# srv/pcl_feature_extraction

Hardware: AMD Instinct MI355X
Metric: Mpoints/s through NARF keypoint + FPFH descriptor on 1M-pt cloud (higher is better)
Workload: dtype f32; 1 GPU; configs[2] 1M-pt synthetic room, NARF(support 0.2) + normals(r 0.05) + FPFH(r 0.08) at the keypoints; image=640x480, parallelism=scan-per-gpu x1, descriptor_rows=83

## Files before the change

### pcl_feature_extraction_amd/csrc/pfx_nblist.hip

```cpp
#include <cstdlib>
#include <cstring>
#include <rocprim/rocprim.hpp>

#include "pfx_nblist.h"
#include "pfx_neighbors.h"

namespace pfx {
namespace {

constexpr int kQ = 16;
typedef float pf2 __attribute__((ext_vector_type(2)));
constexpr int kArena = 16384;
constexpr int kArenaQuery = 16384;
constexpr int kTcapSmall = 384, kTcapSparse = 1280, kTcapDense = 8000;
constexpr int kCapQuery = 4096, kBucketsQuery = 1024;
constexpr int kCapMid8 = 8192, kBucketsMid8 = 1024;
constexpr int kCapMid = 16384, kBucketsMid = 2048;
#ifndef PFX_HUGE_BLOCKS
#define PFX_HUGE_BLOCKS 1024
#endif
constexpr int kCapHuge = 1 << 18, kBucketsHuge = 4096, kHugeBlocks = PFX_HUGE_BLOCKS;
#ifndef PFX_NT_QUERY
#define PFX_NT_QUERY 512
#endif
#ifndef PFX_NT_MID
#define PFX_NT_MID 1024
#endif
#ifndef PFX_NT_MID8
#define PFX_NT_MID8 1024
#endif
#ifndef PFX_Q_PF
#define PFX_Q_PF 1
#endif
#ifndef PFX_Q_WPE
#define PFX_Q_WPE 6
#endif
constexpr int kNtQuery = PFX_NT_QUERY, kNtMid8 = PFX_NT_MID8, kNtMid = PFX_NT_MID, kNtHuge = 256;

enum Counter : int {
  kTilesSmall, kTilesSparse, kTilesDense, kTilesWide,
  kWork4k, kRetryFirst = kWork4k, kWork8k, kWork16k, kWorkHuge,
  kHeadSmall, kHeadSparse, kHeadDense, kHeadWide, kHead4k, kHead8k, kHead16k, kHeadHuge,
  kOverCap,
  kNCounters
};

enum RanTier : int { kRan8k = 1, kRan16k = 2, kRanWide = 4, kRanAll = kRan8k | kRan16k | kRanWide };

constexpr int kCUs = 256;
constexpr int kGridSmall = kCUs * 4 * 2;
constexpr int kGridSparse = kCUs * 3 * 4;
constexpr int kGridDense = kCUs * 2 * 4;
constexpr int kGridWide = kCUs * 4;
constexpr int kGrid4k = kCUs * 4;
constexpr int kGrid8k = kCUs * 2;
constexpr int kGrid16k = kCUs;
constexpr int kGridHugeMax = kHugeBlocks;
constexpr size_t kArenaTails = (size_t)(kGridSmall + kGridSparse + kGridDense) * kArena +
                               (size_t)(kGridWide + kGrid4k + kGrid8k + kGrid16k + kGridHugeMax) * kArenaQuery;

constexpr int32_t kListMode = 1 << 30;
struct TierQ {
  int32_t* q[4];
  int* n[4];
};
__device__ __forceinline__ int query_tier(int k) {
  return k <= kCapQuery ? 0 : (k <= kCapMid8 ? 1 : (k <= kCapMid ? 2 : 3));
}

constexpr int kRecInts = 24;
constexpr int kRecQ0 = 19, kRecQn = 20;

__device__ __forceinline__ void rec_write(int32_t* __restrict__ rec, const Runs& R, int32_t q0, int qn) {
#pragma unroll
  for (int r = 0; r < 9; ++r) rec[r] = R.start[r];
#pragma unroll
  for (int r = 0; r < 10; ++r) rec[9 + r] = R.pref[r];
  rec[kRecQ0] = q0;
  rec[kRecQn] = qn;
}

__device__ __forceinline__ int rec_load(const int32_t* __restrict__ rec_base, int rec_step, int i, bool ok) {
  const int lane = threadIdx.x & 63;
  return (ok && lane < kRecInts) ? rec_base[(int64_t)i * rec_step + lane] : 0;
}
// ... 257 lines not shown
      for (int idx = tid; idx < words; idx += 256) {
        const int tl = idx / kRecInts, w = idx - tl * kRecInts;
        const int32_t v = w < kRecQ0 ? s_runs[s_tcell[tl]][w] : (w == kRecQ0 ? s_tq0[tl] : (w == kRecQn ? s_tqn[tl] : 0));
        recs[(int64_t)s_tat[tl] * kRecInts + w] = v;
      }
      __syncthreads();
    }
  }
}

struct ListOut {
  int64_t* off;
  int32_t* cnt;
  uint8_t* lg;
  uint32_t* list;
  unsigned long long* cursor;
  unsigned long long cap;
  int compact;
  int32_t* qrec;
};

struct CandLds {
  const float2* cxy;
  const float* cz;
  __device__ __forceinline__ void get(int t, float& x, float& y, float& z) const {
    const float2 v = cxy[t];
    x = v.x; y = v.y; z = cz[t];
  }
};
struct CandGlobal {
  const float4* sp;
  const Runs* R;
  __device__ __forceinline__ void get(int t, float& x, float& y, float& z) const {
    const float4 c = sp[run_pos(*R, t)];
    x = c.x; y = c.y; z = c.z;
  }
};

#ifdef PFX_SHOT_PROFILE
constexpr int kTileProbes = 28, kWaveProbes = 12;
__device__ unsigned long long g_tile_prof[kTileProbes];
__device__ unsigned long long g_tile_prof2[kWaveProbes];
#define TPROF_DECL unsigned long long tacc_[kTileProbes] = {}, wacc_[kWaveProbes] = {}
#define TPROF_T(v) long long v = (threadIdx.x == 0) ? clock64() : 0
#define TPROF_ADD(i, a, b) tacc_[i] += (unsigned long long)((b) - (a))
#define WPROF_T(v) long long v = ((threadIdx.x & 63) == 0) ? clock64() : 0
#define WPROF_ADD(i, a, b) wacc_[i] += (unsigned long long)((b) - (a))
#define TPROF_FLUSH                                                                      \
  do {                                                                                   \
    if (threadIdx.x == 0)                                                                \
      _Pragma("unroll") for (int i_ = 0; i_ < kTileProbes; ++i_)                         \
        if (tacc_[i_]) atomicAdd(&g_tile_prof[i_], tacc_[i_]);                           \
    if ((threadIdx.x & 63) == 0)                                                         \
      _Pragma("unroll") for (int i_ = 0; i_ < kWaveProbes; ++i_)                         \
        if (wacc_[i_]) atomicAdd(&g_tile_prof2[i_], wacc_[i_]);                          \
  } while (0)
#else
#define TPROF_DECL
#define TPROF_T(v)
#define TPROF_ADD(i, a, b)
#define WPROF_T(v)
#define WPROF_ADD(i, a, b)
#define TPROF_FLUSH
#endif

template <int NB, int E, class Cand>
__device__ __forceinline__ void wave_sort_regs(uint16_t* L, int k, float qx, float qy, float qz, const Cand& cand,
                                               float bscale, uint32_t* Sd, uint16_t* St, int* bcount, int* bpos,
                                               const GridView& g, const Runs& R, int lane) {
  for (int b = lane; b < NB; b += 64) bcount[b] = 0;
  int t[E], b[E];
  uint32_t d[E];
#pragma unroll
  for (int i = 0; i < E; ++i) t[i] = lane + 64 * i < k ? L[lane + 64 * i] : 0;
  wave_sync();
#pragma unroll
  for (int i = 0; i < E; ++i) {
    float px, py, pz;
    cand.get(t[i], px, py, pz);
    const float d2 = flann_d2(qx, qy, qz, px, py, pz);
    d[i] = __float_as_uint(d2);
    const int bb = (int)(d2 * bscale);
    b[i] = bb < NB ? bb : NB - 1;
    if (lane + 64 * i < k) atomicAdd(&bcount[b[i]], 1);
  }
  wave_sync();
  {
    constexpr int PER = NB / 64;
    int c[PER], sum = 0;
#pragma unroll
    for (int v = 0; v < PER; ++v) { c[v] = bcount[lane * PER + v]; sum += c[v]; }
    const int inc = wave_incl_scan(sum);
    int ex = inc - sum;
#pragma unroll
    for (int v = 0; v < PER; ++v) { bpos[lane * PER + v] = ex; ex += c[v]; }
  }
  wave_sync();
  int slot[E];
#pragma unroll
  for (int i = 0; i < E; ++i) slot[i] = lane + 64 * i < k ? atomicAdd(&bpos[b[i]], 1) : 0;
#pragma unroll
  for (int i = 0; i < E; ++i)
    if (lane + 64 * i < k) {
      Sd[slot[i]] = d[i];
      St[slot[i]] = (uint16_t)t[i];
    }
  wave_sync();
  int st[E], en[E];
#pragma unroll
  for (int i = 0; i < E; ++i) {
    en[i] = bpos[b[i]];
    st[i] = en[i] - bcount[b[i]];
  }
  int rank[E];
  bool tie = false;
#pragma unroll
  for (int i = 0; i < E; ++i) {
    uint32_t dv[4];
#pragma unroll
    for (int j = 0; j < 4; ++j) dv[j] = st[i] + j < en[i] ? Sd[st[i] + j] : 0xffffffffu;
    int r = 0, eq = 0;
#pragma unroll
    for (int j = 0; j < 4; ++j) {
      r += dv[j] < d[i];
      eq += dv[j] == d[i];
    }
    for (int v = st[i] + 4; v < en[i]; ++v) {
      const uint32_t x = Sd[v];
      r += x < d[i];
      eq += x == d[i];
    }
    rank[i] = r;
    tie |= lane + 64 * i < k && eq > 1;
  }
  if (__builtin_amdgcn_ballot_w64(tie)) {
#pragma unroll
    for (int i = 0; i < E; ++i) {
      if (lane + 64 * i >= k) continue;
      const int32_t mine = g.perm[run_pos(R, t[i])];
      for (int v = st[i]; v < en[i]; ++v)
        if (v != slot[i] && Sd[v] == d[i] && g.perm[run_pos(R, St[v])] < mine) ++rank[i];
    }
  }
  wave_sync();
#pragma unroll
  for (int i = 0; i < E; ++i)
    if (lane + 64 * i < k) L[st[i] + rank[i]] = (uint16_t)t[i];
  wave_sync();
}

template <int NB, class Cand>
__device__ __forceinline__ void wave_sort(uint16_t* L, int k, float qx, float qy, float qz, const Cand& cand,
                                          float bscale, uint32_t* Sd, uint16_t* St, int* bcount, int* bpos,
                                          const GridView& g, const Runs& R, int lane) {
  for (int b = lane; b < NB; b += 64) bcount[b] = 0;
  wave_sync();
  for (int e = lane; e < k; e += 64) {
    const int t = L[e];
    float px, py, pz;
    cand.get(t, px, py, pz);
    const int b = (int)(flann_d2(qx, qy, qz, px, py, pz) * bscale);
    atomicAdd(&bcount[b < NB ? b : NB - 1], 1);
  }
  wave_sync();
  {
    constexpr int PER = NB / 64;
    int c[PER], s = 0;
#pragma unroll
    for (int v = 0; v < PER; ++v) { c[v] = bcount[lane * PER + v]; s += c[v]; }
    const int inc = wave_incl_scan(s);
    int ex = inc - s;
#pragma unroll
    for (int v = 0; v < PER; ++v) { bpos[lane * PER + v] = ex; ex += c[v]; }
  }
  wave_sync();
  for (int e = lane; e < k; e += 64) {
    const int t = L[e];
    float px, py, pz;
    cand.get(t, px, py, pz);
    const float d2 = flann_d2(qx, qy, qz, px, py, pz);
    int b = (int)(d2 * bscale);
    b = b < NB ? b : NB - 1;
    const int slot = atomicAdd(&bpos[b], 1);
    Sd[slot] = __float_as_uint(d2);
    St[slot] = (uint16_t)t;
  }
  wave_sync();
  auto bucket_rank = [&](int s, uint32_t d, int t, int st, int en) {
    uint32_t dv[4];
#pragma unroll
    for (int i = 0; i < 4; ++i) dv[i] = st + i < en ? Sd[st + i] : 0xffffffffu;
    int rank = 0;
#pragma unroll
    for (int i = 0; i < 4; ++i) {
      const int v = st + i;
      if (v < en) {
        if (dv[i] < d) ++rank;
        else if (dv[i] == d && v != s && g.perm[run_pos(R, St[v])] < g.perm[run_pos(R, t)]) ++rank;
      }
    }
    for (int v = st + 4; v < en; ++v) {
      const uint32_t x = Sd[v];
      if (x < d) ++rank;
      else if (x == d && v != s && g.perm[run_pos(R, St[v])] < g.perm[run_pos(R, t)]) ++rank;
    }
    return rank;
  };
  for (int s0 = lane; s0 < k; s0 += 128) {
    const int s1 = s0 + 64;
    const bool h1 = s1 < k;
    const uint32_t d0 = Sd[s0], d1 = h1 ? Sd[s1] : 0u;
    const int t0 = St[s0], t1 = h1 ? St[s1] : 0;
    int b0 = (int)(__uint_as_float(d0) * bscale), b1 = (int)(__uint_as_float(d1) * bscale);
    b0 = b0 < NB ? b0 : NB - 1;
    b1 = b1 < NB ? b1 : NB - 1;
    const int en0 = bpos[b0], c0 = bcount[b0], en1 = bpos[b1], c1 = bcount[b1];
    const int st0 = en0 - c0, st1 = en1 - c1;
    const int r0 = bucket_rank(s0, d0, t0, st0, en0);
    const int r1 = h1 ? bucket_rank(s1, d1, t1, st1, en1) : 0;
    L[st0 + r0] = (uint16_t)t0;
    if (h1) L[st1 + r1] = (uint16_t)t1;
  }
  wave_sync();
}

template <class Cand>
__device__ __forceinline__ void wave_rank_sort(uint16_t* L, int k, float qx, float qy, float qz, const Cand& cand,
                                               const GridView& g, const Runs& R, int lane) {
  const bool in = lane < k;
  const int t = in ? L[lane] : 0;
  float px, py, pz;
  cand.get(t, px, py, pz);
  const uint32_t d = in ? __float_as_uint(flann_d2(qx, qy, qz, px, py, pz)) : 0xffffffffu;
  int rank = 0, eq = 0;
  for (int m = 0; m < k; ++m) {
    const uint32_t dm = (uint32_t)__builtin_amdgcn_readlane((int)d, m);
    rank += dm < d ? 1 : 0;
    eq += dm == d ? 1 : 0;
  }
  if (__builtin_amdgcn_ballot_w64(in && eq > 1)) {
    const int32_t id = in ? g.perm[run_pos(R, t)] : 0x7fffffff;
    rank = 0;
    for (int m = 0; m < k; ++m) {
      const uint32_t dm = (uint32_t)__builtin_amdgcn_readlane((int)d, m);
      const int32_t im = __builtin_amdgcn_readlane(id, m);
      rank += (dm < d || (dm == d && im < id)) ? 1 : 0;
    }
  }
  wave_sync();
  if (in) L[rank] = (uint16_t)t;
  wave_sync();
}

template <int NB, class Cand, bool SMALL = false>
__device__ __forceinline__ void sort_list(uint16_t* L, int k, float qx, float qy, float qz, const Cand& cand,
                                          float bscale, uint32_t* Sd, uint16_t* St, int* bcount, int* bpos,
                                          const GridView& g, const Runs& R, int lane) {
  if (k <= 64) wave_rank_sort(L, k, qx, qy, qz, cand, g, R, lane);
  else if (k <= 128) wave_sort_regs<NB, 2>(L, k, qx, qy, qz, cand, bscale, Sd, St, bcount, bpos, g, R, lane);
  else if (k <= 192) wave_sort_regs<NB, 3>(L, k, qx, qy, qz, cand, bscale, Sd, St, bcount, bpos, g, R, lane);
  else if (k <= 256) wave_sort_regs<NB, 4>(L, k, qx, qy, qz, cand, bscale, Sd, St, bcount, bpos, g, R, lane);
  else if (k <= 320) wave_sort_regs<NB, 5>(L, k, qx, qy, qz, cand, bscale, Sd, St, bcount, bpos, g, R, lane);
  else if (SMALL || k <= 384) wave_sort_regs<NB, 6>(L, k, qx, qy, qz, cand, bscale, Sd, St, bcount, bpos, g, R, lane);
  else if (k <= 448) wave_sort_regs<NB, 7>(L, k, qx, qy, qz, cand, bscale, Sd, St, bcount, bpos, g, R, lane);
  else if (k <= 512) wave_sort_regs<NB, 8>(L, k, qx, qy, qz, cand, bscale, Sd, St, bcount, bpos, g, R, lane);
  else if (k <= 640) wave_sort_regs<NB, 10>(L, k, qx, qy, qz, cand, bscale, Sd, St, bcount, bpos, g, R, lane);
  else if (k <= 768) wave_sort_regs<NB, 12>(L, k, qx, qy, qz, cand, bscale, Sd, St, bcount, bpos, g, R, lane);
  else if (k <= 896) wave_sort_regs<NB, 14>(L, k, qx, qy, qz, cand, bscale, Sd, St, bcount, bpos, g, R, lane);
  else if (k <= 1024) wave_sort_regs<NB, 16>(L, k, qx, qy, qz, cand, bscale, Sd, St, bcount, bpos, g, R, lane);
  else wave_sort<NB>(L, k, qx, qy, qz, cand, bscale, Sd, St, bcount, bpos, g, R, lane);
}

__device__ __forceinline__ void push_sort(const TierQ* tq, int32_t j, int k) {
  const int t = query_tier(k);
  tq->q[t][atomicAdd(tq->n[t], 1)] = j | kListMode;
}

constexpr int kChunkWide = 1024;
template <bool STAGE, int SCAP, bool STORE>
__device__ __forceinline__ void tile_pass(const GridView& g, const Runs& R, int T, const float2* cxy, const float* cz,
                                          float2* hxy, float* hz, const pf2* qxy, const float* qz, const bool* act,
                                          const int64_t* gb, int* cursor, uint32_t* __restrict__ glist, float rr) {
  constexpr int CH = kChunkWide, U = 2, QW = 4;
  const int tid = threadIdx.x, lane = tid & 63;
#pragma unroll
  for (int u = 0; u < QW; ++u) cursor[u] = 0;
  float4 cc[STAGE ? 1 : CH / 256];
  if (!STAGE)
#pragma unroll
    for (int u = 0; u < CH / 256; ++u) cc[u] = g.sp[run_pos(R, min(tid + 256 * u, T - 1))];
  for (int c0 = 0; c0 < T; c0 += (STAGE ? T : CH)) {
    const int cend = STAGE ? T : min(T, c0 + CH);
    if (!STAGE) {
      __syncthreads();
#pragma unroll
      for (int u = 0; u < CH / 256; ++u) {
        hxy[tid + 256 * u] = make_float2(cc[u].x, cc[u].y);
        hz[tid + 256 * u] = cc[u].z;
      }
      __syncthreads();
      if (c0 + CH < T)
#pragma unroll
        for (int u = 0; u < CH / 256; ++u) cc[u] = g.sp[run_pos(R, min(c0 + CH + tid + 256 * u, T - 1))];
// ... 35 lines not shown
  }
}

template <int TCAP, bool STAGE>
struct Stager {
  static constexpr int PT = STAGE ? (TCAP + 255) / 256 : 0;
  float x[PT > 0 ? PT : 1], y[PT > 0 ? PT : 1], z[PT > 0 ? PT : 1];
  int32_t qp;
  __device__ __forceinline__ void load(const GridView& g, const int32_t* __restrict__ qpos, const Runs& R,
                                       int32_t start, int qn, bool ok) {
    const int tid = threadIdx.x;
    const int T = ok ? R.pref[9] : 0;
#pragma unroll
    for (int u = 0; u < PT; ++u) {
      const int tc = max(0, min(tid + 256 * u, T - 1));
      const float4 c = g.sp[run_pos(R, tc)];
      x[u] = c.x; y[u] = c.y; z[u] = c.z;
    }
    qp = qpos[start + (tid < qn ? tid : 0)];
  }
  __device__ __forceinline__ void store(float2* cxy, float* cz, int32_t* s_qp, int qn) const {
    const int tid = threadIdx.x;
#pragma unroll
    for (int u = 0; u < PT; ++u) {
      const int t = tid + 256 * u;
      cxy[t] = make_float2(x[u], y[u]);
      cz[t] = z[u];
    }
    if (tid < qn) s_qp[tid] = qp;
  }
};

template <int LCAP, int NB, int TCAP, bool STAGE>
__global__ void __launch_bounds__(256, TCAP <= kTcapSmall ? 4 : (STAGE ? 3 : 2)) k_nb_tile(GridView g, const int32_t* __restrict__ qpos,
                                                 const int32_t* __restrict__ rec_base, int rec_step,
                                                 const int* __restrict__ ntiles_ptr,
                                                 float rr, float bscale, int sorted, ListOut out,
                                                 const TierQ* __restrict__ tq,
                                                 int* __restrict__ next_tile, int chunk) {
  constexpr int Q = kQ, QW = Q / 4;
  constexpr int U = 2;
  constexpr int SCAP = STAGE ? Stager<TCAP, STAGE>::PT * 256 : 1;
  __shared__ float2 cxy[SCAP];
  __shared__ float cz[SCAP];
  constexpr int CH = STAGE ? 1 : 1024;
  __shared__ float2 hxy[CH];
  __shared__ float hz[CH];
  __shared__ uint16_t lists_flat[Q * (LCAP + 2) + 4 * 64];
  uint16_t(*lists)[LCAP + 2] = reinterpret_cast<uint16_t(*)[LCAP + 2]>(lists_flat);
  __shared__ uint32_t sd[4][LCAP];
  __shared__ uint16_t stt[4][LCAP];
  __shared__ int bcount[4][NB], bpos[4][NB];
  __shared__ int s_k[Q];
  __shared__ int32_t s_qp[Q];
  __shared__ unsigned long long s_base;
  __shared__ int s_chunk;
  const int tid = threadIdx.x, lane = tid & 63;
  const int wv = __builtin_amdgcn_readfirstlane(tid >> 6);
  const uint32_t trash_at = (uint32_t)(Q * (LCAP + 2) + 64 * wv + lane);
  const uint32_t wrow = (uint32_t)(wv * (LCAP + 2));
  const int ntiles = *ntiles_ptr;
  TPROF_DECL;
  unsigned long long wg_total = 0, arena_base = 0, arena_left = 0;
  int next_chunk = 0;
  if (tid == 0) {
    s_chunk = atomicAdd(next_tile, chunk);
    next_chunk = atomicAdd(next_tile, chunk);
  }
  __syncthreads();
  int i = __builtin_amdgcn_readfirstlane(s_chunk), i_end = i + chunk;
  Runs R;
  int32_t start = 0;
  int qn = 0;
  {
    const int v = rec_load(rec_base, rec_step, i, i < ntiles);
    rec_unpack(v, R, start, qn);
    Stager<TCAP, STAGE> sg;
    sg.load(g, qpos, R, start, qn, R.pref[9] <= TCAP);
    __syncthreads();
    if (i + 1 == i_end && tid == 0) {
      s_chunk = next_chunk;
      next_chunk = atomicAdd(next_tile, chunk);
    }
    sg.store(cxy, cz, s_qp, qn);
    __syncthreads();
  }
  while (i < ntiles) {
    TPROF_T(p0);
    const int T = R.pref[9];
    const bool ok = T <= TCAP;
    int ni = i + 1;
    if (ni == i_end) {
      ni = __builtin_amdgcn_readfirstlane(s_chunk);
      i_end = ni + chunk;
    }
    const int recv = rec_load(rec_base, rec_step, ni, ni < ntiles);
    pf2 qxy[QW];
    float qz[QW];
    int cursor[QW];
#pragma unroll
    for (int u = 0; u < QW; ++u) {
      const int j = wv + 4 * u;
      cursor[u] = 0;
      qxy[u] = pf2{0.f, 0.f};
      qz[u] = 0.f;
      if (j < qn) {
        const int32_t p = s_qp[j];
        if (STAGE) {
          const int t = R.pref[4] + (p - R.start[4]);
          const float2 v = cxy[t];
          qxy[u] = pf2{v.x, v.y};
          qz[u] = cz[t];
        } else {
          const float4 c = g.sp[p];
          qxy[u] = pf2{c.x, c.y};
          qz[u] = c.z;
        }
      }
    }
    for (int c0 = 0; ok && c0 < T; c0 += (STAGE ? T : CH)) {
      const int cend = STAGE ? T : min(T, c0 + CH);
      if (!STAGE) {
        constexpr int CPT = CH >= 256 ? CH / 256 : 1;
        float4 cc[CPT];
#pragma unroll
        for (int u = 0; u < CPT; ++u) cc[u] = g.sp[run_pos(R, min(c0 + tid + 256 * u, T - 1))];
        __syncthreads();
#pragma unroll
        for (int u = 0; u < CPT; ++u) {
          hxy[tid + 256 * u] = make_float2(cc[u].x, cc[u].y);
          hz[tid + 256 * u] = cc[u].z;
        }
        __syncthreads();
      }
      const float2* XYs = STAGE ? cxy : hxy - c0;
      const float* Zs = STAGE ? cz : hz - c0;
      for (int t0 = c0; t0 < cend; t0 += 64 * U) {
        pf2 pxy[U];
        float pz[U], rrv[U];
#pragma unroll
        for (int v = 0; v < U; ++v) {
          const int t = t0 + 64 * v + lane;
          const int tr = STAGE ? min(t, SCAP - 1) : t;
          const float2 xy = XYs[tr];
          pxy[v] = pf2{xy.x, xy.y};
          pz[v] = Zs[tr];
          rrv[v] = t < cend ? rr : -1.0f;
        }
#pragma unroll
// ... 12 lines not shown
                                                           __builtin_amdgcn_mbcnt_lo((uint32_t)m, (uint32_t)cursor[u]));
            const uint32_t hit_at = (uint32_t)(min(slot, LCAP) + wrow) + (uint32_t)(4 * u * (LCAP + 2));
            const uint32_t sel = 0u - (uint32_t)hit;
            lists_flat[trash_at ^ ((trash_at ^ hit_at) & sel)] = (uint16_t)t;
            cursor[u] += __popcll(m);
          }
        }
      }
    }
    if (lane == 0) {
#pragma unroll
      for (int u = 0; u < QW; ++u)
        if (wv + 4 * u < qn) {
          const int kq = ok ? cursor[u] : LCAP + 1;
          s_k[wv + 4 * u] = kq;
          if (kq > LCAP) qrec_write(out.qrec, start + wv + 4 * u, R, s_qp[wv + 4 * u], qxy[u].x, qxy[u].y, qz[u]);
        }
    }
    __syncthreads();
    TPROF_T(p1);
    TPROF_ADD(TCAP <= kTcapSmall ? 17 : (STAGE ? 1 : 5), p0, p1);
    WPROF_T(ws0);
    [[maybe_unused]] constexpr int kWp0 = TCAP <= kTcapSmall ? 0 : (STAGE ? 4 : 8);
    int lg = 0;
    while ((1 << lg) < qn) ++lg;
    bool c16 = out.compact != 0;
#pragma unroll
    for (int r = 0; r < 9; ++r) c16 = c16 && R.pref[r + 1] - R.pref[r] <= kCompactRun;
    int maxk = 0;
    for (int j = 0; j < qn; ++j) {
      const int k = s_k[j];
      maxk = (k <= LCAP && k > maxk) ? k : maxk;
    }
    if (tid == 0)
      for (int j = 0; j < qn; ++j) wg_total += s_k[j] <= LCAP ? (unsigned long long)s_k[j] : 0ull;
    const unsigned long long need = c16 ? (((unsigned long long)maxk << lg) + 1) >> 1 : (unsigned long long)maxk << lg;
    unsigned long long arena_new = 0, arena_res = 0;
    if (tid == 0 && need > arena_left) {
      arena_res = need > (unsigned long long)kArena ? need : (unsigned long long)kArena;
      arena_new = atomicAdd(out.cursor, arena_res);
    }
    if (tid < qn) {
      const int k = s_k[tid];
      if (k <= LCAP) {
        out.cnt[start + tid] = k;
        out.lg[start + tid] = (uint8_t)(lg | (c16 ? kLgCompact : 0));
      } else {
        const int t = ok ? query_tier(k) : 0;
        if (t == 0) tq->q[0][wave_push_slot(tq->n[0])] = start + tid;
        else tq->q[t][atomicAdd(tq->n[t], 1)] = start + tid;
      }
    }
    if (sorted) {
#pragma unroll
      for (int u = 0; u < QW; ++u) {
        const int j = wv + 4 * u;
        const int k = cursor[u];
        if (ok && j < qn && k <= LCAP && k > 1) {
          if (STAGE) {
            const CandLds cand{cxy, cz};
            sort_list<NB, CandLds, (TCAP <= kTcapSmall)>(lists[j], k, qxy[u].x, qxy[u].y, qz[u], cand, bscale, sd[wv],
                                                         stt[wv], bcount[wv], bpos[wv], g, R, lane);
          } else {
            const CandGlobal cand{g.sp, &R};
            sort_list<NB>(lists[j], k, qxy[u].x, qxy[u].y, qz[u], cand, bscale, sd[wv], stt[wv], bcount[wv], bpos[wv],
                          g, R, lane);
          }
        }
      }
    }
    WPROF_T(ws1);
    WPROF_ADD(kWp0 + 0, ws0, ws1);
    __syncthreads();
    TPROF_T(p2);
    TPROF_ADD(TCAP <= kTcapSmall ? 18 : (STAGE ? 2 : 6), p1, p2);
    WPROF_T(ws2);
    [[maybe_unused]] constexpr int kWp = TCAP <= kTcapSmall ? 0 : (STAGE ? 4 : 8);
    WPROF_ADD(kWp + 1, ws1, ws2);
    Runs Rn;
    int32_t start_n;
    int qn_n;
    rec_unpack(recv, Rn, start_n, qn_n);
    const bool ok_n = ni < ntiles && Rn.pref[9] <= TCAP;
    Stager<TCAP, STAGE> sg;
    if (ni < ntiles) sg.load(g, qpos, Rn, start_n, qn_n, ok_n);
    if (tid == 0) {
      if (ni + 1 == i_end) {
        s_chunk = next_chunk;
        next_chunk = atomicAdd(next_tile, chunk);
      }
      if (arena_res) {
        arena_base = arena_new;
        arena_left = arena_res;
      }
      s_base = arena_base;
      arena_base += need;
      arena_left -= need;
    }
    if (ni < ntiles) sg.store(cxy, cz, s_qp, qn_n);
    WPROF_T(ws3);
    WPROF_ADD(kWp + 2, ws2, ws3);
    __syncthreads();
    WPROF_T(ws4);
    const int64_t base = (int64_t)s_base;
    if (tid < qn && s_k[tid] <= LCAP) out.off[start + tid] = (c16 ? 2 * base : base) + tid;
    const int total = maxk << lg;
    if (c16) {
      const int words = (total + 1) >> 1;
      if ((unsigned long long)(base + words) <= out.cap) {
        for (int w = tid; w < words; w += 256) {
          uint32_t pair = 0;
#pragma unroll
          for (int h = 0; h < 2; ++h) {
            const int e = 2 * w + h;
            const int m = e >> lg, j = e & ((1 << lg) - 1);
            const int k = j < qn ? s_k[j] : 0;
            if (e < total && m < k && k <= LCAP) pair |= (uint32_t)run_entry16(R, lists[j][m]) << (16 * h);
          }
          out.list[base + w] = pair;
        }
      }
    } else if ((unsigned long long)(base + total) <= out.cap) {
      for (int e = tid; e < total; e += 256) {
        const int m = e >> lg, j = e & ((1 << lg) - 1);
        if (j < qn) {
          const int k = s_k[j];
          if (m < k && k <= LCAP) out.list[base + e] = run_entry(R, lists[j][m]);
        }
      }
    }
    WPROF_T(ws5);
    WPROF_ADD(kWp + 3, ws4, ws5);
    __syncthreads();
    TPROF_T(p3);
    TPROF_ADD(TCAP <= kTcapSmall ? 19 : (STAGE ? 3 : 7), p2, p3);
    i = ni;
    R = Rn;
    start = start_n;
    qn = qn_n;
  }
  if (tid == 0 && wg_total) atomicAdd(out.cursor + 1, wg_total);
  TPROF_FLUSH;
}

__global__ void __launch_bounds__(256) k_nb_wide(GridView g, const int32_t* __restrict__ qpos,
                                                 const int32_t* __restrict__ recs, const int32_t* __restrict__ work,
                                                 const int* __restrict__ n_ptr, float rr, int sorted, ListOut out,
                                                 const TierQ* __restrict__ tq, int* __restrict__ next_work) {
  constexpr int QW = 4;
  __shared__ float2 hxy[kChunkWide];
  __shared__ float hz[kChunkWide];
  __shared__ int s_k[kQ];
  __shared__ int32_t s_qp[kQ];
  __shared__ int s_w;
  __shared__ unsigned long long s_base;
  const int tid = threadIdx.x, lane = tid & 63;
  const int wv = __builtin_amdgcn_readfirstlane(tid >> 6);
  const int count = *n_ptr;
  if (count == 0) return;
  unsigned long long wg_total = 0, wg_long = 0, wg_long_n = 0, arena_base = 0, arena_left = 0;
  for (;;) {
    if (tid == 0) s_w = atomicAdd(next_work, 1);
    __syncthreads();
    const int w = __builtin_amdgcn_readfirstlane(s_w);
    __syncthreads();
    if (w >= count) break;
    Runs R;
    int32_t start;
    int qn;
    rec_unpack(rec_load(recs, kRecInts, work[w], true), R, start, qn);
    const int T = R.pref[9];
    if (tid < qn) s_qp[tid] = qpos[start + tid];
    __syncthreads();
    pf2 qxy[QW];
// ... 457 lines not shown
      atomicAdd(out.cursor + 2, wg_long);
      atomicAdd(out.cursor + 3, wg_long_n);
    }
  }
  TPROF_FLUSH;
}

std::string bname(const char* tag, const char* what) { return std::string(tag) + "_" + what; }

struct ListsRb {
  int cnt[kNCounters];
  int oob;
  unsigned long long cur[4];
  int64_t nq;
};

const ListsRb* read_back(pfx_ctx* ctx, const void* counters, const void* cursor, const void* d_nq, const int* oob) {
  hipStream_t st = ctx->stream;
  ListsRb* rb = ctx->readback<ListsRb>();
  PFX_HIP(hipMemcpyAsync(rb->cnt, counters, sizeof(rb->cnt), hipMemcpyDeviceToHost, st));
  PFX_HIP(hipMemcpyAsync(rb->cur, cursor, sizeof(rb->cur), hipMemcpyDeviceToHost, st));
  PFX_HIP(hipMemcpyAsync(&rb->nq, d_nq, sizeof(int64_t), hipMemcpyDeviceToHost, st));
  rb->oob = 0;
  if (oob) PFX_HIP(hipMemcpyAsync(&rb->oob, oob, sizeof(int), hipMemcpyDeviceToHost, st));
  ctx->sync_spin(st);
  return rb;
}

[[noreturn]] void throw_over_cap(const char* tag, int k) {
  throw Error(PFX_ERR_CAPACITY, std::string(tag) + ": a query has " + std::to_string(k) + " neighbours (> " +
                                    std::to_string(kCapHuge) + " supported)");
}

void publish(pfx_ctx* ctx, const char* tag, const ListsRb& rb, size_t list_words, NbLists& out) {
  out.nq = rb.nq;
  out.nq_dev = nullptr;
  out.total = (int64_t)rb.cur[1];
  out.long_total = (int64_t)rb.cur[2];
  out.long_nq = (int64_t)rb.cur[3];
  out.slots = (int64_t)rb.cur[0];
  auto stat = [&](const char* what) -> int64_t& { return ctx->stats[std::string(tag) + what]; };
  stat("_tiles_small") = rb.cnt[kTilesSmall];
  stat("_tiles_sparse") = rb.cnt[kTilesSparse];
  stat("_tiles_dense") = rb.cnt[kTilesDense];
  stat("_wide") = rb.cnt[kTilesWide];
  stat("_single") = rb.cnt[kWork4k];
  stat("_mid8") = rb.cnt[kWork8k];
  stat("_mid") = rb.cnt[kWork16k];
  stat("_huge") = rb.cnt[kWorkHuge];
  stat("_slots") = (int64_t)rb.cur[0];
  stat("_list_words") = (int64_t)list_words;
}

struct TierHint {
  const char* key;
  RanTier bit;
  Counter work;
};
constexpr TierHint kTierHints[3] = {
    {"_hint_mid8", kRan8k, kWork8k}, {"_hint_mid", kRan16k, kWork16k}, {"_hint_wide", kRanWide, kTilesWide}};
int wanted_tiers(pfx_ctx* ctx, const char* tag) {
  int ran = 0;
  for (const TierHint& h : kTierHints) {
    const auto it = ctx->stats.find(std::string(tag) + h.key);
    if (it == ctx->stats.end() || it->second > 0) ran |= h.bit;
  }
  return ran;
}
void note_mid_tiers(pfx_ctx* ctx, const char* tag, const int* h_cnt) {
  for (const TierHint& h : kTierHints) {
    int64_t& v = ctx->stats[std::string(tag) + h.key];
    v = h_cnt[h.work] > 0 ? 16 : std::max<int64_t>(0, v - 1);
  }
}

#ifdef PFX_SHOT_PROFILE
void report_probes(const char* tag) {
  unsigned long long pr[kTileProbes];
  PFX_HIP(hipMemcpyFromSymbol(pr, HIP_SYMBOL(g_tile_prof), sizeof(pr)));
  fprintf(stderr, "%s wave_sort cycles (wave 0): count %llu scan %llu scatter %llu rank %llu\n", tag, pr[8],
          pr[9], pr[10], pr[11]);
  fprintf(stderr, "%s tile cycles: sparse stage %llu test %llu sort %llu write %llu | dense - %llu test %llu "
          "sort %llu write %llu | small - %llu test %llu sort %llu write %llu (cumulative)\n", tag, pr[0], pr[1], pr[2],
          pr[3], pr[4], pr[5], pr[6], pr[7], pr[16], pr[17], pr[18], pr[19]);
  fprintf(stderr, "%s query cycles: test %llu sort+write %llu | entries %llu candidates %llu\n", tag, pr[20],
          pr[21], pr[22], pr[23]);
  fprintf(stderr, "%s query 4k-tier phases: scan %llu scatter %llu rank+write %llu | list-mode items %llu\n", tag,
          pr[24], pr[25], pr[26], pr[27]);
  unsigned long long pw[kWaveProbes];
  PFX_HIP(hipMemcpyFromSymbol(pw, HIP_SYMBOL(g_tile_prof2), sizeof(pw)));
  fprintf(stderr, "%s wave cycles (sum over waves): small sort %llu sortwait %llu staging %llu listwrite %llu | "
          "sparse %llu %llu %llu %llu | dense %llu %llu %llu %llu\n", tag, pw[0], pw[1], pw[2], pw[3], pw[4], pw[5],
          pw[6], pw[7], pw[8], pw[9], pw[10], pw[11]);
  static const unsigned long long zw[kWaveProbes] = {};
  PFX_HIP(hipMemcpyToSymbol(HIP_SYMBOL(g_tile_prof2), zw, sizeof(zw)));
  static const unsigned long long zero[kTileProbes] = {};
  PFX_HIP(hipMemcpyToSymbol(HIP_SYMBOL(g_tile_prof), zero, sizeof(zero)));
}
#endif

struct ListBuild {
  pfx_ctx* ctx;
  const Grid& G;
  const char* tag;
  hipStream_t st;
  const int64_t n;
  const GridView g;
  const float rr;
  const int isort, compact;
  int32_t *qpos, *seg, *tiles, *recs, *wq, *qrec, *cnt;
  int32_t *q4k, *q8k, *q16k, *qhuge;
  int64_t *d_nq, *d_ntiles, *off;
  uint8_t *flags, *lgs;
  int* counters;
  unsigned long long* cursor;
  TierQ* tq_dev;
  size_t t1 = 0, t2 = 0, t3 = 0;
  void* tmp;
  DevBuf &lb, &hs;
  int ch_small, ch_sparse, ch_dense;
  static constexpr size_t kHugeSlice = sizeof(uint32_t) * 4 * (size_t)kCapHuge;

  DevBuf& buf(const char* what) { return ctx->bufs[bname(tag, what)]; }

  ListBuild(pfx_ctx* c, const Grid& grid, const char* t, double radius, bool sorted, bool compact_)
      : ctx(c), G(grid), tag(t), st(c->stream), n(grid.n), g(view(grid)), rr((float)(radius * radius)),
        isort(sorted ? 1 : 0), compact(compact_ ? 1 : 0), lb(buf("list")), hs(buf("scratch")) {
    qpos = buf("qpos").as<int32_t>(n);
    d_nq = buf("nq").as<int64_t>(1);
    flags = buf("flags").as<uint8_t>(n);
// ... 264 lines not shown
```

Baseline: 219.5 Mpoints/s.

## Shrink dense tile LDS and registers to run three workgroups per CU

The dense neighbour-list tile kernel now targets three resident workgroups per CU instead of two. To get there it overlays the list rows, candidate staging and sort scratch in one shared-memory union and drops the separate tag array and bcount/bpos pair in favour of one in-place bucket array. It also adds a lean register-sort variant that recomputes buckets instead of holding them, and moves query coordinates and arena bookkeeping into LDS. The cost is extra recomputation and LDS traffic, plus a riskier in-place sort, in exchange for more latency hiding; the old spill-style wave_sort path is removed and an occupancy query is added to the stats.

New measurement: 229.7 Mpoints/s, median of 6. 4.7% higher.

```diff
diff --git a/pcl_feature_extraction_amd/csrc/pfx_nblist.hip b/pcl_feature_extraction_amd/csrc/pfx_nblist.hip
--- a/pcl_feature_extraction_amd/csrc/pfx_nblist.hip
+++ b/pcl_feature_extraction_amd/csrc/pfx_nblist.hip
@@ -1,5 +1,8 @@
+#include <array>
 #include <cstdlib>
 #include <cstring>
+#include <map>
+#include <mutex>
 #include <rocprim/rocprim.hpp>
 
 #include "pfx_nblist.h"
@@ -35,6 +38,13 @@
 #ifndef PFX_Q_WPE
 #define PFX_Q_WPE 6
 #endif
+#ifndef PFX_DENSE_WG_PER_CU
+#define PFX_DENSE_WG_PER_CU 3
+#endif
+#ifndef PFX_DENSE_ROUNDS
+#define PFX_DENSE_ROUNDS (PFX_DENSE_WG_PER_CU == 2 ? 4 : 2)
+#endif
+static_assert(PFX_DENSE_WG_PER_CU == 2 || PFX_DENSE_WG_PER_CU == 3, "the dense tiles run two or three workgroups per CU");
 constexpr int kNtQuery = PFX_NT_QUERY, kNtMid8 = PFX_NT_MID8, kNtMid = PFX_NT_MID, kNtHuge = 256;
 
 enum Counter : int {
@@ -48,9 +58,10 @@
 enum RanTier : int { kRan8k = 1, kRan16k = 2, kRanWide = 4, kRanAll = kRan8k | kRan16k | kRanWide };
 
 constexpr int kCUs = 256;
-constexpr int kGridSmall = kCUs * 4 * 2;
-constexpr int kGridSparse = kCUs * 3 * 4;
-constexpr int kGridDense = kCUs * 2 * 4;
+constexpr int kWgSmall = 4, kWgSparse = 3, kWgDense = PFX_DENSE_WG_PER_CU;
+constexpr int kGridSmall = kCUs * kWgSmall * 2;
+constexpr int kGridSparse = kCUs * kWgSparse * 4;
+constexpr int kGridDense = kCUs * kWgDense * PFX_DENSE_ROUNDS;
 constexpr int kGridWide = kCUs * 4;
 constexpr int kGrid4k = kCUs * 4;
 constexpr int kGrid8k = kCUs * 2;
@@ -374,7 +385,8 @@
   const float4* sp;
   const Runs* R;
   __device__ __forceinline__ void get(int t, float& x, float& y, float& z) const {
-    const float4 c = sp[run_pos(*R, t)];
+    typedef float pf3 __attribute__((ext_vector_type(3)));
+    const pf3 c = *reinterpret_cast<const pf3*>(sp + run_pos(*R, t));
     x = c.x; y = c.y; z = c.z;
   }
 };
@@ -406,12 +418,18 @@
 #define TPROF_FLUSH
 #endif
 
-template <int NB, int E, class Cand>
+template <int NB, int E, bool LEAN, class Cand>
 __device__ __forceinline__ void wave_sort_regs(uint16_t* L, int k, float qx, float qy, float qz, const Cand& cand,
-                                               float bscale, uint32_t* Sd, uint16_t* St, int* bcount, int* bpos,
-                                               const GridView& g, const Runs& R, int lane) {
-  for (int b = lane; b < NB; b += 64) bcount[b] = 0;
-  int t[E], b[E];
+                                               float bscale, uint32_t* Sd, int* bk, const GridView& g, const Runs& R,
+                                               int lane) {
+  auto bucket_of = [&](uint32_t dbits) {
+    const int bb = (int)(__uint_as_float(dbits) * bscale);
+    return bb < NB ? bb : NB - 1;
+  };
+  constexpr int EH = LEAN ? 1 : E;
+  for (int b = lane; b < NB; b += 64) bk[b] = 0;
+  int t[E];
+  [[maybe_unused]] int bh[EH], slot[EH], st[EH], en[EH];
   uint32_t d[E];
 #pragma unroll
   for (int i = 0; i < E; ++i) t[i] = lane + 64 * i < k ? L[lane + 64 * i] : 0;
@@ -420,149 +438,110 @@
   for (int i = 0; i < E; ++i) {
     float px, py, pz;
     cand.get(t[i], px, py, pz);
-    const float d2 = flann_d2(qx, qy, qz, px, py, pz);
-    d[i] = __float_as_uint(d2);
-    const int bb = (int)(d2 * bscale);
-    b[i] = bb < NB ? bb : NB - 1;
-    if (lane + 64 * i < k) atomicAdd(&bcount[b[i]], 1);
+    d[i] = __float_as_uint(flann_d2(qx, qy, qz, px, py, pz));
+    const int b = bucket_of(d[i]);
+    if constexpr (!LEAN) bh[i] = b;
+    if (lane + 64 * i < k) atomicAdd(&bk[b], 1);
   }
   wave_sync();
   {
     constexpr int PER = NB / 64;
     int c[PER], sum = 0;
 #pragma unroll
-    for (int v = 0; v < PER; ++v) { c[v] = bcount[lane * PER + v]; sum += c[v]; }
+    for (int v = 0; v < PER; ++v) { c[v] = bk[lane * PER + v]; sum += c[v]; }
     const int inc = wave_incl_scan(sum);
     int ex = inc - sum;
 #pragma unroll
-    for (int v = 0; v < PER; ++v) { bpos[lane * PER + v] = ex; ex += c[v]; }
+    for (int v = 0; v < PER; ++v) { bk[lane * PER + v] = ex; ex += c[v]; }
   }
   wave_sync();
-  int slot[E];
-#pragma unroll
-  for (int i = 0; i < E; ++i) slot[i] = lane + 64 * i < k ? atomicAdd(&bpos[b[i]], 1) : 0;
-#pragma unroll
-  for (int i = 0; i < E; ++i)
-    if (lane + 64 * i < k) {
-      Sd[slot[i]] = d[i];
-      St[slot[i]] = (uint16_t)t[i];
-    }
+  if constexpr (LEAN) {
+    int sl[E];
+#pragma unroll
+    for (int i = 0; i < E; ++i) sl[i] = lane + 64 * i < k ? atomicAdd(&bk[bucket_of(d[i])], 1) : 0;
+#pragma unroll
+    for (int i = 0; i < E; ++i)
+      if (lane + 64 * i < k) {
+        Sd[sl[i]] = d[i];
+        L[sl[i]] = (uint16_t)t[i];
+      }
+  } else {
+#pragma unroll
+    for (int i = 0; i < E; ++i) slot[i] = lane + 64 * i < k ? atomicAdd(&bk[bh[i]], 1) : 0;
+#pragma unroll
+    for (int i = 0; i < E; ++i)
+      if (lane + 64 * i < k) {
+        Sd[slot[i]] = d[i];
+        L[slot[i]] = (uint16_t)t[i];
+      }
+  }
   wave_sync();
-  int st[E], en[E];
+  if constexpr (!LEAN) {
+#pragma unroll
+    for (int i = 0; i < E; ++i) {
+      en[i] = bk[bh[i]];
+      const int lo = bk[bh[i] > 0 ? bh[i] - 1 : 0];
+      st[i] = bh[i] > 0 ? lo : 0;
+    }
+  }
+  [[maybe_unused]] int rank[EH];
+  bool tie = false;
 #pragma unroll
   for (int i = 0; i < E; ++i) {
-    en[i] = bpos[b[i]];
-    st[i] = en[i] - bcount[b[i]];
-  }
-  int rank[E];
-  bool tie = false;
-#pragma unroll
-  for (int i = 0; i < E; ++i) {
+    int s0, e0;
+    if constexpr (LEAN) {
+      const int b = bucket_of(d[i]);
+      const int lo = bk[b > 0 ? b - 1 : 0];
+      e0 = bk[b];
+      s0 = b > 0 ? lo : 0;
+    } else {
+      s0 = st[i];
+      e0 = en[i];
+    }
     uint32_t dv[4];
 #pragma unroll
-    for (int j = 0; j < 4; ++j) dv[j] = st[i] + j < en[i] ? Sd[st[i] + j] : 0xffffffffu;
+    for (int j = 0; j < 4; ++j) dv[j] = s0 + j < e0 ? Sd[s0 + j] : 0xffffffffu;
     int r = 0, eq = 0;
 #pragma unroll
     for (int j = 0; j < 4; ++j) {
       r += dv[j] < d[i];
       eq += dv[j] == d[i];
     }
-    for (int v = st[i] + 4; v < en[i]; ++v) {
+    for (int v = s0 + 4; v < e0; ++v) {
       const uint32_t x = Sd[v];
       r += x < d[i];
       eq += x == d[i];
     }
-    rank[i] = r;
+    if constexpr (LEAN) t[i] |= (s0 + r) << 16;
+    else rank[i] = r;
     tie |= lane + 64 * i < k && eq > 1;
   }
   if (__builtin_amdgcn_ballot_w64(tie)) {
 #pragma unroll
     for (int i = 0; i < E; ++i) {
       if (lane + 64 * i >= k) continue;
-      const int32_t mine = g.perm[run_pos(R, t[i])];
-      for (int v = st[i]; v < en[i]; ++v)
-        if (v != slot[i] && Sd[v] == d[i] && g.perm[run_pos(R, St[v])] < mine) ++rank[i];
+      if constexpr (LEAN) {
+        const int b = bucket_of(d[i]);
+        const int e0 = bk[b], s0 = b > 0 ? bk[b - 1] : 0;
+        int ti = t[i] & 0xffff;
+        asm volatile("" : "+v"(ti));
+        const int32_t mine = g.perm[run_pos(R, ti)];
+        for (int v = s0; v < e0; ++v)
+          if (Sd[v] == d[i] && g.perm[run_pos(R, L[v])] < mine) t[i] += 1 << 16;
+      } else {
+        const int32_t mine = g.perm[run_pos(R, t[i])];
+        for (int v = st[i]; v < en[i]; ++v)
+          if (v != slot[i] && Sd[v] == d[i] && g.perm[run_pos(R, L[v])] < mine) ++rank[i];
+      }
     }
   }
   wave_sync();
 #pragma unroll
   for (int i = 0; i < E; ++i)
-    if (lane + 64 * i < k) L[st[i] + rank[i]] = (uint16_t)t[i];
-  wave_sync();
-}
-
-template <int NB, class Cand>
-__device__ __forceinline__ void wave_sort(uint16_t* L, int k, float qx, float qy, float qz, const Cand& cand,
-                                          float bscale, uint32_t* Sd, uint16_t* St, int* bcount, int* bpos,
-                                          const GridView& g, const Runs& R, int lane) {
-  for (int b = lane; b < NB; b += 64) bcount[b] = 0;
-  wave_sync();
-  for (int e = lane; e < k; e += 64) {
-    const int t = L[e];
-    float px, py, pz;
-    cand.get(t, px, py, pz);
-    const int b = (int)(flann_d2(qx, qy, qz, px, py, pz) * bscale);
-    atomicAdd(&bcount[b < NB ? b : NB - 1], 1);
-  }
-  wave_sync();
-  {
-    constexpr int PER = NB / 64;
-    int c[PER], s = 0;
-#pragma unroll
-    for (int v = 0; v < PER; ++v) { c[v] = bcount[lane * PER + v]; s += c[v]; }
-    const int inc = wave_incl_scan(s);
-    int ex = inc - s;
-#pragma unroll
-    for (int v = 0; v < PER; ++v) { bpos[lane * PER + v] = ex; ex += c[v]; }
-  }
-  wave_sync();
-  for (int e = lane; e < k; e += 64) {
-    const int t = L[e];
-    float px, py, pz;
-    cand.get(t, px, py, pz);
-    const float d2 = flann_d2(qx, qy, qz, px, py, pz);
-    int b = (int)(d2 * bscale);
-    b = b < NB ? b : NB - 1;
-    const int slot = atomicAdd(&bpos[b], 1);
-    Sd[slot] = __float_as_uint(d2);
-    St[slot] = (uint16_t)t;
-  }
-  wave_sync();
-  auto bucket_rank = [&](int s, uint32_t d, int t, int st, int en) {
-    uint32_t dv[4];
-#pragma unroll
-    for (int i = 0; i < 4; ++i) dv[i] = st + i < en ? Sd[st + i] : 0xffffffffu;
-    int rank = 0;
-#pragma unroll
-    for (int i = 0; i < 4; ++i) {
-      const int v = st + i;
-      if (v < en) {
-        if (dv[i] < d) ++rank;
-        else if (dv[i] == d && v != s && g.perm[run_pos(R, St[v])] < g.perm[run_pos(R, t)]) ++rank;
-      }
-    }
-    for (int v = st + 4; v < en; ++v) {
-      const uint32_t x = Sd[v];
-      if (x < d) ++rank;
-      else if (x == d && v != s && g.perm[run_pos(R, St[v])] < g.perm[run_pos(R, t)]) ++rank;
-    }
-    return rank;
-  };
-  for (int s0 = lane; s0 < k; s0 += 128) {
-    const int s1 = s0 + 64;
-    const bool h1 = s1 < k;
-    const uint32_t d0 = Sd[s0], d1 = h1 ? Sd[s1] : 0u;
-    const int t0 = St[s0], t1 = h1 ? St[s1] : 0;
-    int b0 = (int)(__uint_as_float(d0) * bscale), b1 = (int)(__uint_as_float(d1) * bscale);
-    b0 = b0 < NB ? b0 : NB - 1;
-    b1 = b1 < NB ? b1 : NB - 1;
-    const int en0 = bpos[b0], c0 = bcount[b0], en1 = bpos[b1], c1 = bcount[b1];
-    const int st0 = en0 - c0, st1 = en1 - c1;
-    const int r0 = bucket_rank(s0, d0, t0, st0, en0);
-    const int r1 = h1 ? bucket_rank(s1, d1, t1, st1, en1) : 0;
-    L[st0 + r0] = (uint16_t)t0;
-    if (h1) L[st1 + r1] = (uint16_t)t1;
-  }
+    if (lane + 64 * i < k) {
+      if constexpr (LEAN) L[t[i] >> 16] = (uint16_t)t[i];
+      else L[st[i] + rank[i]] = (uint16_t)t[i];
+    }
   wave_sync();
 }
 
@@ -594,23 +573,23 @@
   wave_sync();
 }
 
-template <int NB, class Cand, bool SMALL = false>
+template <int NB, class Cand, bool SMALL, bool LEAN>
 __device__ __forceinline__ void sort_list(uint16_t* L, int k, float qx, float qy, float qz, const Cand& cand,
-                                          float bscale, uint32_t* Sd, uint16_t* St, int* bcount, int* bpos,
-                                          const GridView& g, const Runs& R, int lane) {
+                                          float bscale, uint32_t* Sd, int* bk, const GridView& g, const Runs& R,
+                                          int lane) {
+  static_assert(NB % 64 == 0, "the in-place bucket scan takes NB / 64 buckets per lane");
   if (k <= 64) wave_rank_sort(L, k, qx, qy, qz, cand, g, R, lane);
-  else if (k <= 128) wave_sort_regs<NB, 2>(L, k, qx, qy, qz, cand, bscale, Sd, St, bcount, bpos, g, R, lane);
-  else if (k <= 192) wave_sort_regs<NB, 3>(L, k, qx, qy, qz, cand, bscale, Sd, St, bcount, bpos, g, R, lane);
-  else if (k <= 256) wave_sort_regs<NB, 4>(L, k, qx, qy, qz, cand, bscale, Sd, St, bcount, bpos, g, R, lane);
-  else if (k <= 320) wave_sort_regs<NB, 5>(L, k, qx, qy, qz, cand, bscale, Sd, St, bcount, bpos, g, R, lane);
-  else if (SMALL || k <= 384) wave_sort_regs<NB, 6>(L, k, qx, qy, qz, cand, bscale, Sd, St, bcount, bpos, g, R, lane);
-  else if (k <= 448) wave_sort_regs<NB, 7>(L, k, qx, qy, qz, cand, bscale, Sd, St, bcount, bpos, g, R, lane);
-  else if (k <= 512) wave_sort_regs<NB, 8>(L, k, qx, qy, qz, cand, bscale, Sd, St, bcount, bpos, g, R, lane);
-  else if (k <= 640) wave_sort_regs<NB, 10>(L, k, qx, qy, qz, cand, bscale, Sd, St, bcount, bpos, g, R, lane);
-  else if (k <= 768) wave_sort_regs<NB, 12>(L, k, qx, qy, qz, cand, bscale, Sd, St, bcount, bpos, g, R, lane);
-  else if (k <= 896) wave_sort_regs<NB, 14>(L, k, qx, qy, qz, cand, bscale, Sd, St, bcount, bpos, g, R, lane);
-  else if (k <= 1024) wave_sort_regs<NB, 16>(L, k, qx, qy, qz, cand, bscale, Sd, St, bcount, bpos, g, R, lane);
-  else wave_sort<NB>(L, k, qx, qy, qz, cand, bscale, Sd, St, bcount, bpos, g, R, lane);
+  else if (k <= 128) wave_sort_regs<NB, 2, LEAN>(L, k, qx, qy, qz, cand, bscale, Sd, bk, g, R, lane);
+  else if (k <= 192) wave_sort_regs<NB, 3, LEAN>(L, k, qx, qy, qz, cand, bscale, Sd, bk, g, R, lane);
+  else if (k <= 256) wave_sort_regs<NB, 4, LEAN>(L, k, qx, qy, qz, cand, bscale, Sd, bk, g, R, lane);
+  else if (k <= 320) wave_sort_regs<NB, 5, LEAN>(L, k, qx, qy, qz, cand, bscale, Sd, bk, g, R, lane);
+  else if (SMALL || k <= 384) wave_sort_regs<NB, 6, LEAN>(L, k, qx, qy, qz, cand, bscale, Sd, bk, g, R, lane);
+  else if (k <= 448) wave_sort_regs<NB, 7, LEAN>(L, k, qx, qy, qz, cand, bscale, Sd, bk, g, R, lane);
+  else if (k <= 512) wave_sort_regs<NB, 8, LEAN>(L, k, qx, qy, qz, cand, bscale, Sd, bk, g, R, lane);
+  else if (k <= 640) wave_sort_regs<NB, 10, LEAN>(L, k, qx, qy, qz, cand, bscale, Sd, bk, g, R, lane);
+  else if (k <= 768) wave_sort_regs<NB, 12, LEAN>(L, k, qx, qy, qz, cand, bscale, Sd, bk, g, R, lane);
+  else if (k <= 896) wave_sort_regs<NB, 14, LEAN>(L, k, qx, qy, qz, cand, bscale, Sd, bk, g, R, lane);
+  else wave_sort_regs<NB, 16, LEAN>(L, k, qx, qy, qz, cand, bscale, Sd, bk, g, R, lane);
 }
 
 __device__ __forceinline__ void push_sort(const TierQ* tq, int32_t j, int k) {
@@ -712,7 +691,7 @@
 };
 
 template <int LCAP, int NB, int TCAP, bool STAGE>
-__global__ void __launch_bounds__(256, TCAP <= kTcapSmall ? 4 : (STAGE ? 3 : 2)) k_nb_tile(GridView g, const int32_t* __restrict__ qpos,
+__global__ void __launch_bounds__(256, TCAP <= kTcapSmall ? kWgSmall : (STAGE ? kWgSparse : kWgDense)) k_nb_tile(GridView g, const int32_t* __restrict__ qpos,
                                                  const int32_t* __restrict__ rec_base, int rec_step,
                                                  const int* __restrict__ ntiles_ptr,
                                                  float rr, float bscale, int sorted, ListOut out,
@@ -723,17 +702,24 @@
   constexpr int SCAP = STAGE ? Stager<TCAP, STAGE>::PT * 256 : 1;
   __shared__ float2 cxy[SCAP];
   __shared__ float cz[SCAP];
-  constexpr int CH = STAGE ? 1 : 1024;
-  __shared__ float2 hxy[CH];
-  __shared__ float hz[CH];
-  __shared__ uint16_t lists_flat[Q * (LCAP + 2) + 4 * 64];
-  uint16_t(*lists)[LCAP + 2] = reinterpret_cast<uint16_t(*)[LCAP + 2]>(lists_flat);
-  __shared__ uint32_t sd[4][LCAP];
-  __shared__ uint16_t stt[4][LCAP];
-  __shared__ int bcount[4][NB], bpos[4][NB];
+  constexpr int CH = STAGE ? 0 : 1024;
+  static_assert(LCAP <= 1024, "sort_list's last register tier holds 1024 entries");
+  constexpr int kRowBytes = Q * (LCAP + 2) * (int)sizeof(uint16_t);
+  constexpr int kTrashBytes = 4 * 64 * (int)sizeof(uint16_t);
+  constexpr int kTestBytes = kTrashBytes + CH * (int)(sizeof(float2) + sizeof(float));
+  constexpr int kSortBytes = 4 * (LCAP * (int)sizeof(uint32_t) + NB * (int)sizeof(int));
+  static_assert(kRowBytes % 16 == 0 && kTrashBytes % 16 == 0, "the views start 16-byte aligned");
+  __shared__ __attribute__((aligned(16))) unsigned char s_raw[kRowBytes + (kTestBytes > kSortBytes ? kTestBytes : kSortBytes)];
+  uint16_t* lists_flat = reinterpret_cast<uint16_t*>(s_raw);
+  uint16_t(*lists)[LCAP + 2] = reinterpret_cast<uint16_t(*)[LCAP + 2]>(s_raw);
+  [[maybe_unused]] float2* hxy = reinterpret_cast<float2*>(s_raw + kRowBytes + kTrashBytes);
+  [[maybe_unused]] float* hz = reinterpret_cast<float*>(s_raw + kRowBytes + kTrashBytes + CH * (int)sizeof(float2));
+  uint32_t(*sd)[LCAP] = reinterpret_cast<uint32_t(*)[LCAP]>(s_raw + kRowBytes);
+  int(*bk)[NB] = reinterpret_cast<int(*)[NB]>(s_raw + kRowBytes + 4 * LCAP * (int)sizeof(uint32_t));
   __shared__ int s_k[Q];
   __shared__ int32_t s_qp[Q];
-  __shared__ unsigned long long s_base;
+  __shared__ float s_q[STAGE ? 1 : Q][3];
+  __shared__ unsigned long long s_base, s_wg_total, s_arena_base, s_arena_left;
   __shared__ int s_chunk;
   const int tid = threadIdx.x, lane = tid & 63;
   const int wv = __builtin_amdgcn_readfirstlane(tid >> 6);
@@ -741,9 +727,14 @@
   const uint32_t wrow = (uint32_t)(wv * (LCAP + 2));
   const int ntiles = *ntiles_ptr;
   TPROF_DECL;
-  unsigned long long wg_total = 0, arena_base = 0, arena_left = 0;
+  [[maybe_unused]] unsigned long long r_wg_total = 0, r_arena_base = 0, r_arena_left = 0;
   int next_chunk = 0;
   if (tid == 0) {
+    if (!STAGE) {
+      s_wg_total = 0;
+      s_arena_base = 0;
+      s_arena_left = 0;
+    }
     s_chunk = atomicAdd(next_tile, chunk);
     next_chunk = atomicAdd(next_tile, chunk);
   }
@@ -795,6 +786,11 @@
           const float4 c = g.sp[p];
           qxy[u] = pf2{c.x, c.y};
           qz[u] = c.z;
+          if (lane == 0) {
+            s_q[j][0] = c.x;
+            s_q[j][1] = c.y;
+            s_q[j][2] = c.z;
+          }
         }
       }
     }
@@ -873,12 +869,18 @@
       const int k = s_k[j];
       maxk = (k <= LCAP && k > maxk) ? k : maxk;
     }
-    if (tid == 0)
-      for (int j = 0; j < qn; ++j) wg_total += s_k[j] <= LCAP ? (unsigned long long)s_k[j] : 0ull;
+    if (tid == 0) {
+      unsigned long long sum = 0;
+      for (int j = 0; j < qn; ++j) sum += s_k[j] <= LCAP ? (unsigned long long)s_k[j] : 0ull;
+      if (STAGE) r_wg_total += sum;
+      else s_wg_total += sum;
+    }
     const unsigned long long need = c16 ? (((unsigned long long)maxk << lg) + 1) >> 1 : (unsigned long long)maxk << lg;
-    unsigned long long arena_new = 0, arena_res = 0;
-    if (tid == 0 && need > arena_left) {
-      arena_res = need > (unsigned long long)kArena ? need : (unsigned long long)kArena;
+    const unsigned long long arena_res = need > (unsigned long long)kArena ? need : (unsigned long long)kArena;
+    unsigned long long arena_new = 0;
+    bool reserved = false;
+    if (tid == 0 && need > (STAGE ? r_arena_left : s_arena_left)) {
+      reserved = true;
       arena_new = atomicAdd(out.cursor, arena_res);
     }
     if (tid < qn) {
@@ -896,16 +898,15 @@
 #pragma unroll
       for (int u = 0; u < QW; ++u) {
         const int j = wv + 4 * u;
-        const int k = cursor[u];
+        const int k = STAGE ? cursor[u] : __builtin_amdgcn_readfirstlane(j < qn ? s_k[j] : 0);
         if (ok && j < qn && k <= LCAP && k > 1) {
           if (STAGE) {
             const CandLds cand{cxy, cz};
-            sort_list<NB, CandLds, (TCAP <= kTcapSmall)>(lists[j], k, qxy[u].x, qxy[u].y, qz[u], cand, bscale, sd[wv],
-                                                         stt[wv], bcount[wv], bpos[wv], g, R, lane);
+            sort_list<NB, CandLds, (TCAP <= kTcapSmall), false>(lists[j], k, qxy[u].x, qxy[u].y, qz[u], cand, bscale, sd[wv],
+                                                         bk[wv], g, R, lane);
           } else {
             const CandGlobal cand{g.sp, &R};
-            sort_list<NB>(lists[j], k, qxy[u].x, qxy[u].y, qz[u], cand, bscale, sd[wv], stt[wv], bcount[wv], bpos[wv],
-                          g, R, lane);
+            sort_list<NB, CandGlobal, false, true>(lists[j], k, s_q[j][0], s_q[j][1], s_q[j][2], cand, bscale, sd[wv], bk[wv], g, R, lane);
           }
         }
       }
@@ -930,13 +931,16 @@
         s_chunk = next_chunk;
         next_chunk = atomicAdd(next_tile, chunk);
       }
-      if (arena_res) {
-        arena_base = arena_new;
-        arena_left = arena_res;
-      }
-      s_base = arena_base;
-      arena_base += need;
-      arena_left -= need;
+      const unsigned long long abase = reserved ? arena_new : (STAGE ? r_arena_base : s_arena_base);
+      const unsigned long long aleft = reserved ? arena_res : (STAGE ? r_arena_left : s_arena_left);
+      s_base = abase;
+      if (STAGE) {
+        r_arena_base = abase + need;
+        r_arena_left = aleft - need;
+      } else {
+        s_arena_base = abase + need;
+        s_arena_left = aleft - need;
+      }
     }
     if (ni < ntiles) sg.store(cxy, cz, s_qp, qn_n);
     WPROF_T(ws3);
@@ -980,7 +984,10 @@
     start = start_n;
     qn = qn_n;
   }
-  if (tid == 0 && wg_total) atomicAdd(out.cursor + 1, wg_total);
+  if (tid == 0) {
+    const unsigned long long total = STAGE ? r_wg_total : s_wg_total;
+    if (total) atomicAdd(out.cursor + 1, total);
+  }
   TPROF_FLUSH;
 }
 
@@ -1504,6 +1511,26 @@
                                     std::to_string(kCapHuge) + " supported)");
 }
 
+void tile_residency(int wg[3]) {
+  static std::mutex mu;
+  static std::map<int, std::array<int, 3>> cache;
+  int dev = 0;
+  PFX_HIP(hipGetDevice(&dev));
+  std::lock_guard<std::mutex> lock(mu);
+  auto it = cache.find(dev);
+  if (it == cache.end()) {
+    std::array<int, 3> a{};
+    PFX_HIP(hipOccupancyMaxActiveBlocksPerMultiprocessor(
+        &a[0], (const void*)k_nb_tile<kTcapSmall, 256, kTcapSmall, true>, 256, 0));
+    PFX_HIP(hipOccupancyMaxActiveBlocksPerMultiprocessor(
+        &a[1], (const void*)k_nb_tile<512, 256, kTcapSparse, true>, 256, 0));
+    PFX_HIP(hipOccupancyMaxActiveBlocksPerMultiprocessor(
+        &a[2], (const void*)k_nb_tile<1024, 256, kTcapDense, false>, 256, 0));
+    it = cache.emplace(dev, a).first;
+  }
+  for (int c = 0; c < 3; ++c) wg[c] = it->second[c];
+}
+
 void publish(pfx_ctx* ctx, const char* tag, const ListsRb& rb, size_t list_words, NbLists& out) {
   out.nq = rb.nq;
   out.nq_dev = nullptr;
@@ -1520,6 +1547,11 @@
   stat("_mid8") = rb.cnt[kWork8k];
   stat("_mid") = rb.cnt[kWork16k];
   stat("_huge") = rb.cnt[kWorkHuge];
+  int wg[3];
+  tile_residency(wg);
+  stat("_tile_wg_per_cu_small") = wg[0];
+  stat("_tile_wg_per_cu_sparse") = wg[1];
+  stat("_tile_wg_per_cu_dense") = wg[2];
   stat("_slots") = (int64_t)rb.cur[0];
   stat("_list_words") = (int64_t)list_words;
 }
@@ -1564,10 +1596,10 @@
   fprintf(stderr, "%s wave cycles (sum over waves): small sort %llu sortwait %llu staging %llu listwrite %llu | "
           "sparse %llu %llu %llu %llu | dense %llu %llu %llu %llu\n", tag, pw[0], pw[1], pw[2], pw[3], pw[4], pw[5],
           pw[6], pw[7], pw[8], pw[9], pw[10], pw[11]);
-  static const unsigned long long zw[kWaveProbes] = {};
-  PFX_HIP(hipMemcpyToSymbol(HIP_SYMBOL(g_tile_prof2), zw, sizeof(zw)));
-  static const unsigned long long zero[kTileProbes] = {};
-  PFX_HIP(hipMemcpyToSymbol(HIP_SYMBOL(g_tile_prof), zero, sizeof(zero)));
+  static const unsigned long long zw[sizeof(g_tile_prof2) / sizeof(unsigned long long)] = {};
+  PFX_HIP(hipMemcpyToSymbol(HIP_SYMBOL(g_tile_prof2), zw, sizeof(g_tile_prof2)));
+  static const unsigned long long zero[sizeof(g_tile_prof) / sizeof(unsigned long long)] = {};
+  PFX_HIP(hipMemcpyToSymbol(HIP_SYMBOL(g_tile_prof), zero, sizeof(g_tile_prof)));
 }
 #endif
 
```
